# ylongqi/openrec

Measured on NVIDIA H100. Metric: bpr_triplets_per_sec, higher is better.
Workload: dtype f32

## Files before the change

### openrec_b200/csrc/orx_common.cuh

```cuda
#pragma once
#include <cuda_runtime.h>
#include <stdint.h>
#include <stdio.h>

#include <functional>
#include <initializer_list>
#include <type_traits>

#include "../../include/orx.h"

void orx_set_error(const char* fmt, ...);

#define ORX_CUDA(call)                                                                         \
  do {                                                                                         \
    cudaError_t e__ = (call);                                                                  \
    if (e__ != cudaSuccess) {                                                                  \
      orx_set_error("%s:%d %s -> %s", __FILE__, __LINE__, #call, cudaGetErrorString(e__));     \
      return ORX_ERR_CUDA;                                                                     \
    }                                                                                          \
  } while (0)

#define ORX_REQUIRE(cond, msg)                                  \
  do {                                                          \
    if (!(cond)) {                                              \
// ... 237 lines not shown
  return r;
}
__device__ __forceinline__ float orx_rcp_fast(float x) {
  float r;
  asm("rcp.approx.f32 %0, %1;" : "=f"(r) : "f"(x));
  return r;
}

template <int OPT>
struct OrxOptSlots {
  static constexpr bool S0 = (OPT == ORX_OPT_ADAGRAD || OPT == ORX_OPT_ADAM_LAZY);
  static constexpr bool S1 = (OPT == ORX_OPT_ADAM_LAZY);
  static constexpr bool STAGE_ONLY = (OPT == ORX_OPT_ADAM_DENSE);
};

template <int OPT>
__device__ __forceinline__ float orx_apply(float w, float g, float& s0, float& s1, const OrxOptDev& o) {
  if (OPT == ORX_OPT_SGD) {
    return w - o.lr * g;
  } else if (OPT == ORX_OPT_ADAGRAD) {
    s0 = s0 + g * g;
    return w - o.lr * g * orx_rcp_fast(orx_sqrt_fast(s0) + o.eps);
  } else {
    s0 = o.beta1 * s0 + (1.f - o.beta1) * g;
    s1 = o.beta2 * s1 + (1.f - o.beta2) * g * g;
    return w - o.lr * s0 * orx_rcp_fast(orx_sqrt_fast(s1) + o.eps);
  }
}

template <int OPT>
__device__ __forceinline__ float4 orx_apply4(float4 w, float4 g, float4& s0, float4& s1, const OrxOptDev& o) {
  float4 r;
  r.x = orx_apply<OPT>(w.x, g.x, s0.x, s1.x, o);
  r.y = orx_apply<OPT>(w.y, g.y, s0.y, s1.y, o);
  r.z = orx_apply<OPT>(w.z, g.z, s0.z, s1.z, o);
  r.w = orx_apply<OPT>(w.w, g.w, s0.w, s1.w, o);
  return r;
}

template <int OPT, bool STREAM>
__device__ __forceinline__ void orx_own_or_stage4(bool own, float* W, float* P0, float* P1, int id, float* G, int d,
                                                  int D, int off, float4 w, float4 g, float4& s0, float4& s1,
                                                  const OrxOptDev& o) {
  typedef OrxOptSlots<OPT> SL;
  auto st = [](float* p, float4 v) {
    if (STREAM) orx_st4_stream(p, v);
    else __stcg(reinterpret_cast<float4*>(p), v);
  };
  if (!SL::STAGE_ONLY && own) {
    const int64_t i = (int64_t)id * D + off;
    st(W + i, orx_apply4<OPT>(w, g, s0, s1, o));
    if (SL::S0) st(P0 + i, s0);
    if (SL::S1) st(P1 + i, s1);
  } else {
    orx_red4(G + (int64_t)d * D + off, g);
  }
}

template <int OPT>
__device__ __forceinline__ void orx_update1(float* W, float* P0, float* P1, float w, float g, const OrxOptDev& o) {
  typedef OrxOptSlots<OPT> SL;
  float s0 = SL::S0 ? *P0 : 0.f, s1 = SL::S1 ? *P1 : 0.f;
  *W = orx_apply<OPT>(w, g, s0, s1, o);
  if (SL::S0) *P0 = s0;
  if (SL::S1) *P1 = s1;
}

__device__ __forceinline__ void orx_adam_dense1(float* W, float* M, float* V, int64_t i, float g, const OrxOptDev& o) {
  const float mm = o.beta1 * M[i] + (1.f - o.beta1) * g;
  const float vv = o.beta2 * V[i] + (1.f - o.beta2) * g * g;
  M[i] = mm;
  V[i] = vv;
  W[i] = W[i] - o.lr * mm / (sqrtf(vv) + o.eps);
}

__device__ __forceinline__ void orx_block_partial(float loss, float l2, float* partials) {
  __shared__ float sred[8][2];
  loss = orx_group_sum<32>(loss);
  l2 = orx_group_sum<32>(l2);
  if ((threadIdx.x & 31) == 0) {
    sred[threadIdx.x >> 5][0] = loss;
    sred[threadIdx.x >> 5][1] = l2;
  }
  __syncthreads();
  if (threadIdx.x == 0) {
    float l = 0.f, q = 0.f;
#pragma unroll
    for (int w = 0; w < 8; ++w) {
      l += sred[w][0];
      q += sred[w][1];
    }
    partials[2 * blockIdx.x] = l;
    partials[2 * blockIdx.x + 1] = q;
  }
}

__device__ __forceinline__ void orx_warp_partial(float loss, float l2, float* partials) {
  const int warp = (blockIdx.x * blockDim.x + threadIdx.x) >> 5;
  loss = orx_group_sum<32>(loss);
  l2 = orx_group_sum<32>(l2);
  if ((threadIdx.x & 31) == 0) {
    partials[2 * warp] = loss;
    partials[2 * warp + 1] = l2;
  }
}

__device__ __forceinline__ void orx_block_sum_partials(const float* partials, int n, const float* sq, int nsq,
                                                       double* l, double* q) {
  __shared__ double sh[2][256];
  double sl = 0.0, sq2 = 0.0;
  for (int i = threadIdx.x; i < n; i += blockDim.x) {
    sl += (double)__ldcg(partials + 2 * i);
    sq2 += (double)__ldcg(partials + 2 * i + 1);
  }
  if (sq)
    for (int e = threadIdx.x; e < nsq; e += blockDim.x) sq2 += (double)sq[e] * (double)sq[e];
  sh[0][threadIdx.x] = sl;
  sh[1][threadIdx.x] = sq2;
  __syncthreads();
  for (int s = 128; s > 0; s >>= 1) {
    if ((int)threadIdx.x < s) {
      sh[0][threadIdx.x] += sh[0][threadIdx.x + s];
      sh[1][threadIdx.x] += sh[1][threadIdx.x + s];
    }
    __syncthreads();
  }
  *l = sh[0][0];
  *q = sh[1][0];
}

#endif

struct SparseArgs {
  float *U, *Us0, *Us1;
  float *I, *Is0, *Is1;
  float *Bv, *Bs0, *Bs1;
  float *gu, *gi, *gb;
  OrxHash hu, hi;
  OrxOptDev opt;
  int D;
};

struct TailArgs : SparseArgs {
  const float* partials;
  int n_partials;
  float loss_scale;
  int32_t* counters;
  float* out4;
  float *W, *Ws0, *Ws1, *gw;
  float c_l2;
};

#ifdef __CUDACC__
template <int OPT>
__device__ __forceinline__ void orx_tail_rows(const TailArgs& a, int nu, int ni) {
  typedef OrxOptSlots<OPT> SL;
  constexpr bool ZERO_ONLY = SL::STAGE_ONLY;
  const int lane = threadIdx.x & 31;
  const int gwarp = (blockIdx.x * blockDim.x + threadIdx.x) >> 5;
  const int nwarps = (gridDim.x * blockDim.x) >> 5;
  const int D = a.D;
  const float4 z4 = make_float4(0.f, 0.f, 0.f, 0.f);
  const int sub = lane >> 3, sl = lane & 7;
  for (int r0 = gwarp * 4; r0 < nu + ni; r0 += nwarps * 4) {
    const int r = r0 + sub;
    const bool on = r < nu + ni;
    const bool is_u = on && r < nu;
    const int d = on ? (is_u ? r : r - nu) : 0;
    const int id = on ? (is_u ? a.hu.did[d] : a.hi.did[d]) : 0;
    float* G = (is_u ? a.gu : a.gi) + (int64_t)d * D;
    float* W = (is_u ? a.U : a.I) + (int64_t)id * D;
    float* P0 = (is_u ? a.Us0 : a.Is0) + (int64_t)id * D;
    float* P1 = (is_u ? a.Us1 : a.Is1) + (int64_t)id * D;
    if ((D & 3) == 0) {
      const int nq = D >> 2;
      for (int e0 = 0; e0 < nq; e0 += 32) {
        float4 g[4], w[4], s0v[4], s1v[4];
#pragma unroll
        for (int k = 0; k < 4; ++k) {
          const int e = e0 + sl + 8 * k;
          const bool ld = on && e < nq;
          g[k] = ld ? __ldcg(reinterpret_cast<const float4*>(G) + e) : z4;
          w[k] = (ld && !ZERO_ONLY) ? orx_ld4_stream(W + 4 * e) : z4;
          s0v[k] = (ld && SL::S0) ? orx_ld4_stream(P0 + 4 * e) : z4;
          s1v[k] = (ld && SL::S1) ? orx_ld4_stream(P1 + 4 * e) : z4;
        }
#pragma unroll
        for (int k = 0; k < 4; ++k) {
          const int e = e0 + sl + 8 * k;
          if (!on || e >= nq) continue;
          if (!ZERO_ONLY) {
            orx_st4_stream(W + 4 * e, orx_apply4<OPT>(w[k], g[k], s0v[k], s1v[k], a.opt));
            if (SL::S0) orx_st4_stream(P0 + 4 * e, s0v[k]);
            if (SL::S1) orx_st4_stream(P1 + 4 * e, s1v[k]);
          }
          __stcg(reinterpret_cast<float4*>(G) + e, z4);
        }
      }
    } else if (on) {
      for (int e = sl; e < D; e += 8) {
        if (!ZERO_ONLY) orx_update1<OPT>(W + e, P0 + e, P1 + e, W[e], G[e], a.opt);
        G[e] = 0.f;
      }
    }
    if (on && !is_u && sl == 0) {
      if (!ZERO_ONLY) orx_update1<OPT>(a.Bv + id, a.Bs0 + id, a.Bs1 + id, a.Bv[id], a.gb[d], a.opt);
      a.gb[d] = 0.f;
    }
  }
}
#endif

OrxOptDev orx_opt_to_dev(const orx_opt_t* o);
int orx_launch_index_build_strided(orx_ctx* c, const int32_t* a, int64_t stride, int64_t rows, int32_t n,
                                   bool stage_all, cudaStream_t st);
SparseArgs orx_sparse_args(const orx_ctx* c, const orx_table_t* user, const orx_table_t* item, const orx_table_t* bias,
                           const OrxHash& hu, const OrxHash& hi, const OrxOptDev& o);
int orx_check_step_tables(const orx_table_t* user, const orx_table_t* item, const orx_table_t* bias,
                          const orx_table_t* w, int opt_kind);
static inline int orx_step_blocks(int B) { return ((B + 7) / 8 + 7) / 8; }
struct OrxStepLaunch {
  int n_partials, variant, minb;
};
typedef std::function<int(const SparseArgs& s, float* partials, OrxStepLaunch* out)> OrxStepKernel;
int orx_sparse_step(orx_ctx* c, int op, int kind, const orx_table_t* user, const orx_table_t* item,
                    const orx_table_t* bias, const orx_table_t* w, const int32_t* uid, const int32_t* iid,
                    const int32_t* nid, int B, const orx_opt_t* opt, float loss_scale, float c_l2, float* out4,
                    const OrxStepKernel& kernel, cudaStream_t st);
int orx_sparse_unfused(orx_ctx* c, int B, float loss_scale, float* out4,
                       const std::function<void(float* partials, int blocks)>& launch, cudaStream_t st);
int orx_launch_adam_sweeps(orx_ctx* c, const orx_table_t* user, const orx_table_t* item, const orx_table_t* bias,
                           const OrxHash& hu, const OrxHash& hi, const OrxOptDev& o, cudaStream_t st);
int orx_launch_tail(orx_ctx* c, const TailArgs& ta, int opt_kind, cudaStream_t st);
int orx_launch_reduce_partials(const float* partials, int n, float loss_scale, float* out4, cudaStream_t st);
int orx_launch_index_build(orx_ctx* c, const int32_t* a, int64_t rows_a, const int32_t* b0, const int32_t* b1,
                           int64_t rows_b, int32_t n, int mode , cudaStream_t st);
```

### openrec_b200/csrc/orx_pairwise.cu

```cuda
#include "orx_common.cuh"
#include "orx_pair.cuh"

__global__ void k_index_build(OrxHash hu, OrxHash hi, const int32_t* __restrict__ a, int64_t rows_a,
                              const int32_t* __restrict__ b0, const int32_t* __restrict__ b1, int64_t rows_b, int n,
                              int stage_all, int32_t* bad) {
  const int i = blockIdx.x * blockDim.x + threadIdx.x;
  if (i >= (b1 ? 3 : 2) * n) return;
  const int t = i < n ? i : (i < 2 * n ? i - n : i - 2 * n);
  const int32_t ia = a[t], ib0 = b0[t], ib1 = b1 ? b1[t] : 0;
  const bool ga = ia >= 0 && (int64_t)ia < rows_a, gb0 = ib0 >= 0 && (int64_t)ib0 < rows_b,
             gb1 = ib1 >= 0 && (int64_t)ib1 < rows_b;
  const bool all = ga && gb0 && gb1;
  if (i < n) {
    if (!ga) atomicAdd(bad, 1);
    else if (all) orx_hash_insert(hu, ia, stage_all);
  } else {
    const bool g = i < 2 * n ? gb0 : gb1;
    if (!g) atomicAdd(bad, 1);
    else if (all) orx_hash_insert(hi, i < 2 * n ? ib0 : ib1, stage_all);
  }
}

__global__ void k_index_build_strided(OrxHash hu, const int32_t* __restrict__ a, int64_t stride, int64_t rows, int n,
                                       int stage_all, int32_t* bad) {
// ... 186 lines not shown
  } else {
#pragma unroll 1
    for (int j = 0; j < CH; j += TPW) {
      if (j > 0) {
        load_var(j, ra);
        load_slots(j, ra);
      }
      process(j, ra);
    }
  }

  orx_pdl_trigger();
  if (flags & 1) {
    if (flags & 4) {
      __stcg(a.Bv + p_id, orx_apply<OPT>(bp, g_own, bps0, bps1, a.opt));
      if (SL::S0) __stcg(a.Bs0 + p_id, bps0);
      if (SL::S1) __stcg(a.Bs1 + p_id, bps1);
    } else {
      atomicAdd(a.gb + dp, g_own);
    }
    if (flags & 8) {
      __stcg(a.Bv + n_id, orx_apply<OPT>(bn, -g_own, bns0, bns1, a.opt));
      if (SL::S0) __stcg(a.Bs0 + n_id, bns0);
      if (SL::S1) __stcg(a.Bs1 + n_id, bns1);
    } else {
      atomicAdd(a.gb + dn, -g_own);
    }
  }

  orx_block_partial(loss_acc, l2_acc, a.partials);
}

template <int KIND, int OPT, int MODE>
__global__ void __launch_bounds__(256) k_pair_generic(const PairArgs a) {
  constexpr bool STAGE_ONLY = OrxOptSlots<OPT>::STAGE_ONLY;
  const int lane = threadIdx.x & 31;
  const int warp = (blockIdx.x * blockDim.x + threadIdx.x) >> 5;
  const int D = a.D;
  const bool row_form = MODE == 1 && a.ld != 0;
  const int64_t ld = row_form ? a.ld : D;
  float loss_acc = 0.f, l2_acc = 0.f;
  orx_pdl_wait();
  for (int j = 0; j < 8; ++j) {
    const int t = warp * 8 + j;
    if (t >= a.B) break;
    const int uu = a.uid[t], pp = a.pid[t], nn = a.nid[t];
    const bool ok = uu >= 0 && uu < a.rowsU && pp >= 0 && pp < a.rowsI && nn >= 0 && nn < a.rowsI;
    float* ur = a.U + (int64_t)uu * ld;
    float* pr = a.I + (int64_t)pp * ld;
    float* nr = a.I + (int64_t)nn * ld;
    float s1 = 0.f, s2 = 0.f, sq = 0.f, bp = 0.f, bn = 0.f, lt = 0.f, g = 0.f;
    if (ok) {
      for (int d = lane; d < D; d += 32) {
        const float u = ur[d], p = pr[d], n = nr[d];
        if (KIND == ORX_PAIR_BPR) {
          s1 += u * p;
          s2 += u * n;
        } else {
          s1 += (u - p) * (u - p);
          s2 += (u - n) * (u - n);
        }
        sq += u * u + p * p + n * n;
      }
      bp = row_form ? pr[D] : a.Bv[pp];
      bn = row_form ? nr[D] : a.Bv[nn];
    }
    l2_acc += sq;
    s1 = orx_group_sum<32>(s1);
    s2 = orx_group_sum<32>(s2);
    if (ok) pair_score<KIND>(s1, s2, bp, bn, a.margin, a.c_loss, a.inv_B, &lt, &g);
    if (lane == 0) loss_acc += lt;
    const float gbias = (KIND == ORX_PAIR_BPR) ? g : -g;
    if (MODE == 0) {
      if (!ok) continue;
      int du, dp, dn;
      const uint32_t cu = orx_hash_find<!STAGE_ONLY>(a.hu, uu, &du);
      const uint32_t cp = orx_hash_find<!STAGE_ONLY>(a.hi, pp, &dp);
      const uint32_t cn = orx_hash_find<!STAGE_ONLY>(a.hi, nn, &dn);
      const bool fu = !STAGE_ONLY && cu == 1u, fp = !STAGE_ONLY && cp == 1u, fn = !STAGE_ONLY && cn == 1u;
      for (int d = lane; d < D; d += 32) {
        const float u = ur[d], p = pr[d], n = nr[d];
        float gu, gp, gn;
        pair_grads1<KIND>(g, a.c_l2, u, p, n, &gu, &gp, &gn);
        const int64_t ou = (int64_t)uu * D + d, op = (int64_t)pp * D + d, on = (int64_t)nn * D + d;
        if (fu) orx_update1<OPT>(ur + d, a.Us0 + ou, a.Us1 + ou, u, gu, a.opt);
        else atomicAdd(a.gu + (int64_t)du * D + d, gu);
        if (fp) orx_update1<OPT>(pr + d, a.Is0 + op, a.Is1 + op, p, gp, a.opt);
        else atomicAdd(a.gi + (int64_t)dp * D + d, gp);
        if (fn) orx_update1<OPT>(nr + d, a.Is0 + on, a.Is1 + on, n, gn, a.opt);
        else atomicAdd(a.gi + (int64_t)dn * D + d, gn);
      }
      if (lane == 0) {
        if (fp) orx_update1<OPT>(a.Bv + pp, a.Bs0 + pp, a.Bs1 + pp, bp, gbias, a.opt);
        else atomicAdd(a.gb + dp, gbias);
        if (fn) orx_update1<OPT>(a.Bv + nn, a.Bs0 + nn, a.Bs1 + nn, bn, -gbias, a.opt);
        else atomicAdd(a.gb + dn, -gbias);
      }
      continue;
    }
    if (a.d_user || a.d_pos || a.d_neg) {
      for (int d = lane; d < D; d += 32) {
        float gu = 0.f, gp = 0.f, gn = 0.f;
        if (ok) pair_grads1<KIND>(g, a.c_l2, ur[d], pr[d], nr[d], &gu, &gp, &gn);
        if (row_form) {
          if (ok) {
            a.d_user[(int64_t)uu * ld + d] = gu;
            a.d_pos[(int64_t)pp * ld + d] = gp;
            a.d_neg[(int64_t)nn * ld + d] = gn;
          }
        } else {
          const int64_t o = (int64_t)t * D + d;
          if (a.d_user) a.d_user[o] = gu;
          if (a.d_pos) a.d_pos[o] = gp;
          if (a.d_neg) a.d_neg[o] = gn;
        }
      }
    }
    if (lane == 0) {
      if (row_form) {
        if (ok) {
          for (int64_t c = D; c < ld; ++c) {
            a.d_user[(int64_t)uu * ld + c] = 0.f;
            a.d_pos[(int64_t)pp * ld + c] = c == D ? gbias : 0.f;
            a.d_neg[(int64_t)nn * ld + c] = c == D ? -gbias : 0.f;
          }
        }
      } else {
        if (a.d_bp) a.d_bp[t] = gbias;
        if (a.d_bn) a.d_bn[t] = -gbias;
      }
      if (a.g_out) a.g_out[t] = g;
    }
  }
  orx_warp_partial(loss_acc, l2_acc, a.partials);
}

__global__ void __launch_bounds__(256) k_adam_sweep(float* var, float* m, float* v, int64_t rows, int D, OrxHash h,
                                                    const float* gstage, OrxOptDev o) {
  const int lane = threadIdx.x & 31;
  const int64_t nw = ((int64_t)gridDim.x * blockDim.x) >> 5;
  for (int64_t r = ((int64_t)blockIdx.x * blockDim.x + threadIdx.x) >> 5; r < rows; r += nw) {
    int d = -1;
    uint32_t c = 0;
    if (lane == 0) c = orx_hash_find(h, (int32_t)r, &d);
    c = __shfl_sync(ORX_FULL, c, 0);
    d = __shfl_sync(ORX_FULL, d, 0);
    for (int e = lane; e < D; e += 32)
      orx_adam_dense1(var, m, v, r * D + e, c ? gstage[(int64_t)d * D + e] : 0.f, o);
  }
}


template <int OPT>
__global__ void __launch_bounds__(256) k_sparse_tail(const TailArgs a) {
  __shared__ bool last;
  orx_pdl_wait();
  const int nu = *a.hu.counter, ni = a.I ? *a.hi.counter : 0;
  orx_tail_rows<OPT>(a, nu, ni);

  if (blockIdx.x == 0 && a.out4) {
    double l, q;
    orx_block_sum_partials(a.partials, a.n_partials, a.W, a.W ? a.D : 0, &l, &q);
    if (threadIdx.x == 0) {
      a.out4[0] = (float)(l * (double)a.loss_scale);
      a.out4[1] = (float)(0.5 * q);
      a.out4[2] = (float)a.counters[3];
      a.out4[3] = (float)(nu + ni);
    }
    if (a.W) {
      for (int e = threadIdx.x; e < a.D; e += blockDim.x) {
        const float g = a.gw[e] + a.c_l2 * a.W[e];
        if (OrxOptSlots<OPT>::STAGE_ONLY) orx_adam_dense1(a.W, a.Ws0, a.Ws1, e, g, a.opt);
        else orx_update1<OPT>(a.W + e, a.Ws0 + e, a.Ws1 + e, a.W[e], g, a.opt);
        a.gw[e] = 0.f;
      }
    }
  }
  __syncthreads();
  if (threadIdx.x == 0) {
    __threadfence();
    const int tk = atomicAdd(a.counters + 2, 1);
    last = (tk == (int)gridDim.x - 1);
  }
  __syncthreads();
  if (last && threadIdx.x < 4) a.counters[threadIdx.x] = 0;
}

int orx_launch_tail(orx_ctx* c, const TailArgs& ta, int opt_kind, cudaStream_t st) {
  const int grid = c->num_sms * 4;
  orx_dispatch_opt(opt_kind, [&](auto O) {
    orx_launch_pdl(k_sparse_tail<decltype(O)::value>, dim3(grid), dim3(256), 0, st, ta);
  });
  ORX_LAUNCH_CHECK();
  return ORX_OK;
}

int orx_launch_adam_sweeps(orx_ctx* c, const orx_table_t* user, const orx_table_t* item, const orx_table_t* bias,
                           const OrxHash& hu, const OrxHash& hi, const OrxOptDev& o, cudaStream_t st) {
  struct { const orx_table_t* t; int D; const OrxHash* h; const float* g; } sw[3] = {
      {user, user->dim, &hu, c->gu}, {item, user->dim, &hi, c->gi}, {bias, 1, &hi, c->gb}};
  for (const auto& s : sw) {
    if (!s.t) continue;
    int64_t blocks = (s.t->rows + 7) / 8;
    const int64_t cap = (int64_t)c->num_sms * 16;
    if (blocks > cap) blocks = cap;
    if (blocks < 1) blocks = 1;
    k_adam_sweep<<<(int)blocks, 256, 0, st>>>(s.t->var, s.t->s0, s.t->s1, s.t->rows, s.D, *s.h, s.g, o);
    ORX_LAUNCH_CHECK();
  }
  return ORX_OK;
}

SparseArgs orx_sparse_args(const orx_ctx* c, const orx_table_t* user, const orx_table_t* item, const orx_table_t* bias,
                           const OrxHash& hu, const OrxHash& hi, const OrxOptDev& o) {
  SparseArgs s = {};
  s.U = user->var; s.Us0 = user->s0; s.Us1 = user->s1;
  if (item) { s.I = item->var; s.Is0 = item->s0; s.Is1 = item->s1; }
  if (bias) { s.Bv = bias->var; s.Bs0 = bias->s0; s.Bs1 = bias->s1; }
  s.D = user->dim; s.opt = o; s.hu = hu; s.hi = hi;
  s.gu = c->gu; s.gi = c->gi; s.gb = c->gb;
  return s;
}

int orx_check_step_tables(const orx_table_t* user, const orx_table_t* item, const orx_table_t* bias,
                          const orx_table_t* w, int opt_kind) {
  ORX_REQUIRE(user && item && bias, "null table");
  ORX_REQUIRE(user->var && item->var && bias->var, "null table storage");
  ORX_REQUIRE(user->dim == item->dim && user->dim > 0, "user/item dims must match and be positive");
  ORX_REQUIRE(bias->dim == 1 && bias->rows == item->rows, "item_bias must be [item.rows, 1]");
  ORX_REQUIRE(user->rows > 0 && item->rows > 0 && user->rows <= 0x7fffffffLL && item->rows <= 0x7fffffffLL,
              "row counts must fit int32 ids");
  ORX_REQUIRE(!w || (w->var && w->dim == user->dim), "GMF needs w with dim == D");
  ORX_REQUIRE(orx_opt_slots_ok(opt_kind, {user, item, bias, w}), "optimizer slot rows missing");
  return ORX_OK;
}

template <int KIND, int OPT>
static int launch_pair_step_kind_opt(const PairArgs& pa, cudaStream_t st, OrxStepLaunch* out) {
  constexpr bool LAZY = (OPT == ORX_OPT_ADAM_LAZY);
  const int blocks = orx_step_blocks(pa.B);
  auto go = [&](auto kern, int variant, int minb, int n_partials) {
    *out = {n_partials, variant, minb};
    orx_launch_pdl(kern, dim3(blocks), dim3(256), 0, st, pa);
  };
  constexpr int PV = LAZY ? ORX_VARIANT_STEP : ORX_VARIANT_STEP_PIPE;
  switch (pa.D) {
    case 32: go(k_pair_step<KIND, OPT, 32, 8, 2, !LAZY>, PV, 2, blocks); break;
    case 64: go(k_pair_step<KIND, OPT, 64, 8, 2, !LAZY>, PV, 2, blocks); break;
    case 128:
      if constexpr (LAZY) go(k_pair_step<KIND, OPT, 128, 8, 3, false>, ORX_VARIANT_STEP, 3, blocks);
      else go(k_pair_step<KIND, OPT, 128, 8, 4, false>, ORX_VARIANT_STEP, 4, blocks);
      break;
    case 256: go(k_pair_step<KIND, OPT, 256, 8, 2, !LAZY>, PV, 2, blocks); break;
    default: go(k_pair_generic<KIND, OPT, 0>, ORX_VARIANT_STEP_GENERIC, 0, 8 * blocks); break;
  }
  ORX_LAUNCH_CHECK();
  return ORX_OK;
}

static int side_stream_ensure(orx_ctx* c) {
  if (c->side_stream) return ORX_OK;
  ORX_CUDA(cudaStreamCreateWithFlags(&c->side_stream, cudaStreamNonBlocking));
  ORX_CUDA(cudaEventCreateWithFlags(&c->side_ev, cudaEventDisableTiming));
  for (int i = 0; i < 2; ++i) {
    ORX_CUDA(cudaEventCreateWithFlags(&c->pf_done[i], cudaEventDisableTiming));
    ORX_CUDA(cudaEventCreateWithFlags(&c->pf_free[i], cudaEventDisableTiming));
    ORX_CUDA(cudaEventCreateWithFlags(&c->stage_free[i], cudaEventDisableTiming));
    c->pf_free_valid[i] = c->stage_free_valid[i] = 0;
  }
  return ORX_OK;
}

static int prefetch_drop(orx_ctx* c, cudaStream_t st) {
  if (!c->pf_valid) return ORX_OK;
  const int k = c->pf_set;
  ORX_CUDA(cudaStreamWaitEvent(st, c->pf_done[k], 0));
  ORX_CUDA(cudaMemsetAsync(c->counters + 4 * (1 + k), 0, sizeof(int32_t) * 4, st));
  ORX_CUDA(cudaEventRecord(c->pf_free[k], st));
  c->pf_free_valid[k] = 1;
  c->pf_valid = 0;
  return ORX_OK;
}

static int prefetch_issue(orx_ctx* c, const int32_t* uid, const int32_t* pid, const int32_t* nid, int B, int64_t rows_u,
                          int64_t rows_i, int mode) {
  const int k = c->pf_next;
  c->pf_next ^= 1;
  cudaStream_t ss = c->side_stream;
  if (c->pf_free_valid[k]) ORX_CUDA(cudaStreamWaitEvent(ss, c->pf_free[k], 0));
  int rc = orx_next_epoch(c, ss);
  if (rc) return rc;
  c->pf_u[k].epoch = c->pf_i[k].epoch = c->epoch;
  k_index_build<<<(3 * B + 255) / 256, 256, 0, ss>>>(c->pf_u[k], c->pf_i[k], uid, rows_u, pid, nid, rows_i, B, mode,
                                                     c->counters + 4 * (1 + k) + 3);
  ORX_LAUNCH_CHECK();
  ORX_CUDA(cudaEventRecord(c->pf_done[k], ss));
  c->pf_valid = 1; c->pf_set = k; c->pf_uid = uid; c->pf_pid = pid; c->pf_nid = nid; c->pf_B = B;
  c->pf_rows_u = rows_u; c->pf_rows_i = rows_i; c->pf_mode = mode;
  return ORX_OK;
}

extern "C" int orx_pairwise_prefetch(orx_handle_t h, const orx_table_t* user, const orx_table_t* item, const int32_t* uid,
                                     const int32_t* pid, const int32_t* nid, int32_t B, int32_t opt_kind, int32_t ids_ready,
                                     orx_stream_t ids_stream) {
  ORX_REQUIRE(h != nullptr && user && item && uid && pid && nid && B > 0, "bad arguments");
  ORX_REQUIRE(orx_opt_kind_ok(opt_kind), "unknown optimizer kind");
  ORX_REQUIRE(!orx_shard_holds_index(h), "a sharded step's announced batch holds this handle's index sets (a prefetch "
                                         "would overwrite one) until its orx_shard_step call");
  ORX_CUDA(cudaSetDevice(h->device));
  cudaStream_t is = (cudaStream_t)ids_stream;
  int rc = orx_ensure_workspace(h, B, user->dim);
  if (rc) return rc;
  if ((rc = side_stream_ensure(h))) return rc;
  if ((rc = prefetch_drop(h, is))) return rc;
  if (!ids_ready) {
    ORX_CUDA(cudaEventRecord(h->side_ev, is));
    ORX_CUDA(cudaStreamWaitEvent(h->side_stream, h->side_ev, 0));
  }
  return prefetch_issue(h, uid, pid, nid, B, user->rows, item->rows, opt_kind == ORX_OPT_ADAM_DENSE ? 1 : 0);
}

int orx_sparse_step(orx_ctx* c, int op, int kind, const orx_table_t* user, const orx_table_t* item,
                    const orx_table_t* bias, const orx_table_t* w, const int32_t* uid, const int32_t* iid,
                    const int32_t* nid, int B, const orx_opt_t* opt, float loss_scale, float c_l2, float* out4,
                    const OrxStepKernel& kernel, cudaStream_t st) {
  ORX_REQUIRE(opt != nullptr && out4 != nullptr, "null opt/out");
  ORX_REQUIRE(orx_opt_kind_ok(opt->kind), "unknown optimizer kind");
  ORX_REQUIRE(B > 0 && uid && iid, "empty batch or null ids");
  int rc = orx_check_step_tables(user, item, bias, w, opt->kind);
  if (rc) return rc;
  const int D = user->dim;
  if ((rc = orx_ensure_workspace(c, B, D))) return rc;
  const bool dense = opt->kind == ORX_OPT_ADAM_DENSE;
  if ((rc = orx_grow((void**)&c->partials, &c->partials_cap, sizeof(float) * 2 * 8 * (size_t)orx_step_blocks(B))))
    return rc;
  orx_prof_mark(c, 0, st);
  int set = 0;
  if (nid && c->pf_valid && c->pf_uid == uid && c->pf_pid == iid && c->pf_nid == nid && c->pf_B == B &&
      c->pf_rows_u == user->rows && c->pf_rows_i == item->rows && c->pf_mode == (dense ? 1 : 0)) {
    set = 1 + c->pf_set;
    ORX_CUDA(cudaStreamWaitEvent(st, c->pf_done[c->pf_set], 0));
    c->pf_valid = 0;
  } else {
    if (nid && (rc = prefetch_drop(c, st))) return rc;
// ... 189 lines not shown
```

### openrec_b200/csrc/orx_shard.cu

```cuda
#include <stdlib.h>
#include <string.h>

#include "orx_common.cuh"
#include "orx_pair.cuh"

#define SH_MAX_R 64
#define SH_META 16
#define SH_NPH 4
#define SH_ERR_WORD (SH_NPH * SH_MAX_R)
#define SH_IDX_BITS 24

enum { SH_M_TRIPS = 0,
       SH_M_REQS = 1,
       SH_M_GOTOFF = 2,
       SH_M_GINBASE = 3,
       SH_M_LOSS = 4, SH_M_L2 = 5 };

enum { SH_C_CURH = 0, SH_C_CURO = SH_MAX_R, SH_C_GOFF = 2 * SH_MAX_R, SH_C_RCO = 3 * SH_MAX_R + 1,
       SH_C_DONE = 4 * SH_MAX_R + 1, SH_C_T = SH_C_DONE + 8, SH_C_NREQ = SH_C_T + 1, SH_C_ACUR = SH_C_T + 2,
       SH_C_BAD = SH_C_T + 4 , SH_C_WORDS = SH_C_T + 8 };

struct ShardHost {
  int32_t world, rank, dim, batch_cap, home_cap, req_cap, gin_cap, timeout_ms;
  void *tripbox, *idbox, *got, *gotb, *gin, *ginb, *meta, *flags;
// ... 424 lines not shown
        }
        sq += dot4(u[k][q], u[k][q]) + dot4(p[k][q], p[k][q]) + dot4(n[k][q], n[k][q]);
      }
      l2_acc += sq;
      s1 = orx_group_sum<32>(s1);
      s2 = orx_group_sum<32>(s2);
      const float bp = __shfl_sync(ORX_FULL, my_bp, k), bn = __shfl_sync(ORX_FULL, my_bn, k);
      float lt, g;
      pair_score<KIND>(s1, s2, bp, bn, a.margin, a.c_loss, a.inv_B, &lt, &g);
      if (lane == 0) loss_acc += lt;
      const int own = __shfl_sync(ORX_FULL, my_own, k);
      const int du = __shfl_sync(ORX_FULL, my_du, k);
      float* dp = reinterpret_cast<float*>(__shfl_sync(ORX_FULL, (unsigned long long)my_dp, k));
      float* dn = reinterpret_cast<float*>(__shfl_sync(ORX_FULL, (unsigned long long)my_dn, k));
      const int pp = __shfl_sync(ORX_FULL, my_pp, k), pn = __shfl_sync(ORX_FULL, my_pn, k);
#pragma unroll
      for (int q = 0; q < NQ; ++q) {
        const int e = q * 32 + lane;
        if (e >= nq) continue;
        float4 gu, gp, gn;
        pair_row_grads<KIND>(g, a.c_l2, u[k][q], p[k][q], n[k][q], &gu, &gp, &gn);
        if (dp) reinterpret_cast<float4*>(dp)[e] = gp;
        if (dn) reinterpret_cast<float4*>(dn)[e] = gn;
        orx_own_or_stage4<OPT, false>(own, a.U, a.Us0, a.Us1, uu[k], a.gu, du, D, 4 * e, u[k][q], gu, us0[k][q],
                                      us1[k][q], a.opt);
      }
      {
        float* bdp = reinterpret_cast<float*>(__shfl_sync(ORX_FULL, (unsigned long long)my_bdp, k));
        float* bdn = reinterpret_cast<float*>(__shfl_sync(ORX_FULL, (unsigned long long)my_bdn, k));
        const float gb = (KIND == ORX_PAIR_BPR) ? g : -g;
        if (lane == 0) {
          if (bdp) *bdp = gb;
          if (bdn) *bdn = -gb;
        }
      }
    }
  }
  orx_pdl_trigger();
  orx_warp_partial(loss_acc, l2_acc, a.partials);
  sh_arrive(x, w.ctl + SH_C_DONE + 3, gridDim.x, 3, epoch, [&]() {
    double l, q;
    orx_block_sum_partials(a.partials, (int)((gridDim.x * blockDim.x) >> 5), nullptr, 0, &l, &q);
    if ((int)threadIdx.x < R) {
      int32_t* m = x.meta[threadIdx.x] + SH_META * me;
      m[SH_M_LOSS] = __float_as_int((float)(l * (double)a.loss_scale));
      m[SH_M_L2] = __float_as_int((float)(0.5 * q));
    }
  });
}

struct ShApplyArgs {
  float *I, *Is0, *Is1;
  float *Bv, *Bs0, *Bs1;
  OrxHash hi;
  float *gi, *gb;
  OrxOptDev opt;
};

struct ShProArgs {
  int n_route, n_request;
  int epoch;
  ShRouteArgs r;
  OrxHash hu;
};

template <int OPT, int NQ>
__global__ void __launch_bounds__(256) k_sh_apply(ShardDev x, ShardWs w, ShApplyArgs a, ShProArgs pro, int epoch) {
  typedef OrxOptSlots<OPT> SL;
  constexpr int GRP = NQ == 1 ? 4 : (NQ == 2 ? 2 : 1);
  const int me = x.rank, D = x.D, nq = D >> 2;
  orx_pdl_wait();
  if ((int)blockIdx.x < pro.n_route) {
    sh_route_role(x, w, pro.r, pro.epoch, blockIdx.x, pro.n_route);
    orx_pdl_trigger();
    return;
  }
  if ((int)blockIdx.x < pro.n_route + pro.n_request) {
    sh_request_role(x, w, pro.hu, pro.epoch, blockIdx.x - pro.n_route, pro.n_request);
    orx_pdl_trigger();
    return;
  }
  sh_wait(x, 3, epoch);
  const int n = w.ctl[SH_C_NREQ];
  const int lane = threadIdx.x & 31, wid = threadIdx.x >> 5;
  const float* gin = x.gin[me];
  const float* ginb = x.ginb[me];
  const float4 z4 = make_float4(0.f, 0.f, 0.f, 0.f);
  __shared__ int chunk_sh;
  while (true) {
    __syncthreads();
    if (threadIdx.x == 0) chunk_sh = atomicAdd(w.ctl + SH_C_ACUR, 1);
    __syncthreads();
    const int j0 = chunk_sh * 64 + wid * 8;
    if (chunk_sh * 64 >= n) break;
    if (j0 >= n) continue;
    int32_t my_id = -1;
    int my_d = -1, my_own = 0;
    if (lane < 8) {
      my_id = w.req[j0 + lane];
      if (my_id >= 0) {
        my_own = orx_hash_find(a.hi, my_id, &my_d) == 1u;
        const float gbv = __ldcg(ginb + j0 + lane);
        if (my_own) {
          float s0v = SL::S0 ? __ldcg(a.Bs0 + my_id) : 0.f, s1v = SL::S1 ? __ldcg(a.Bs1 + my_id) : 0.f;
          __stcg(a.Bv + my_id, orx_apply<OPT>(__ldcg(a.Bv + my_id), gbv, s0v, s1v, a.opt));
          if (SL::S0) __stcg(a.Bs0 + my_id, s0v);
          if (SL::S1) __stcg(a.Bs1 + my_id, s1v);
        } else {
          atomicAdd(a.gb + my_d, gbv);
        }
      }
    }
    if (__ballot_sync(ORX_FULL, my_id >= 0) == 0u) continue;
#pragma unroll
    for (int k0 = 0; k0 < 8; k0 += GRP) {
      float4 g[GRP][NQ], wv[GRP][NQ], s0v[GRP][NQ], s1v[GRP][NQ];
      int id[GRP], own[GRP], d[GRP];
#pragma unroll
      for (int k = 0; k < GRP; ++k) {
        id[k] = __shfl_sync(ORX_FULL, my_id, k0 + k);
        own[k] = __shfl_sync(ORX_FULL, my_own, k0 + k);
        d[k] = __shfl_sync(ORX_FULL, my_d, k0 + k);
#pragma unroll
        for (int q = 0; q < NQ; ++q) {
          const int e = q * 32 + lane;
          const bool on = id[k] >= 0 && e < nq;
          g[k][q] = on ? __ldcg(reinterpret_cast<const float4*>(gin + (int64_t)(j0 + k0 + k) * D) + e) : z4;
          const bool ld = on && own[k];
          wv[k][q] = ld ? __ldcg(reinterpret_cast<const float4*>(a.I + (int64_t)id[k] * D) + e) : z4;
          s0v[k][q] = (SL::S0 && ld) ? __ldcg(reinterpret_cast<const float4*>(a.Is0 + (int64_t)id[k] * D) + e) : z4;
          s1v[k][q] = (SL::S1 && ld) ? __ldcg(reinterpret_cast<const float4*>(a.Is1 + (int64_t)id[k] * D) + e) : z4;
        }
      }
#pragma unroll
      for (int k = 0; k < GRP; ++k) {
        if (id[k] < 0) continue;
#pragma unroll
        for (int q = 0; q < NQ; ++q) {
          const int e = q * 32 + lane;
          if (e >= nq) continue;
          orx_own_or_stage4<OPT, false>(own[k], a.I, a.Is0, a.Is1, id[k], a.gi, d[k], D, 4 * e, wv[k][q], g[k][q],
                                        s0v[k][q], s1v[k][q], a.opt);
        }
      }
    }
  }
  orx_pdl_trigger();
}

template <int OPT>
__global__ void __launch_bounds__(256) k_sh_tail(ShardDev x, ShardWs w, TailArgs a, int par) {
  orx_pdl_wait();
  const int nu = *a.hu.counter, ni = *a.hi.counter;
  orx_tail_rows<OPT>(a, nu, ni);
  if (blockIdx.x == 0 && threadIdx.x == 0) {
    const int32_t* m = x.meta[x.rank];
    float l = 0.f, q = 0.f;
    for (int r = 0; r < x.world; ++r) {
      l += __int_as_float(__ldcg(m + SH_META * r + SH_M_LOSS));
      q += __int_as_float(__ldcg(m + SH_META * r + SH_M_L2));
    }
    a.out4[0] = l;
    a.out4[1] = q;
    a.out4[2] = (float)w.ctl[SH_C_BAD + par];
    a.out4[3] = (float)(nu + ni);
    w.ctl[SH_C_BAD + par] = 0;
    w.ctl[SH_C_ACUR] = 0;
  }
  __shared__ bool last;
  __syncthreads();
  if (threadIdx.x == 0) {
    __threadfence();
    last = (atomicAdd(a.counters + 2, 1) == (int)gridDim.x - 1);
  }
  __syncthreads();
  if (last && threadIdx.x == 0) {
    *a.hu.counter = 0;
    *a.hi.counter = 0;
    a.counters[2] = 0;
  }
}

struct orx_shard_ws {
  ShardWs w;
  int home_cap, gin_cap, got_rows;
  const void* occ_fn[32];
  int occ[32], n_occ;
  int32_t pro_route[2], pro_request[2];
  uint32_t ep_u[2], ep_i[2];
  const int32_t *ids_u[2], *ids_p[2], *ids_n[2];
  int32_t ids_B[2];
  int32_t serve_epoch, tail_epoch;
  const void* owner;
};

extern "C" int orx_peer_alloc(orx_handle_t h, int64_t bytes, void** dev_ptr_out, uint8_t* handle_out64) {
  ORX_REQUIRE(h != nullptr && dev_ptr_out && handle_out64 && bytes > 0, "bad arguments");
  ORX_CUDA(cudaSetDevice(h->device));
  void* p = nullptr;
  ORX_CUDA(cudaMalloc(&p, (size_t)bytes));
  ORX_CUDA(cudaMemset(p, 0, (size_t)bytes));
  ORX_CUDA(cudaDeviceSynchronize());
  cudaIpcMemHandle_t hd;
  static_assert(sizeof(cudaIpcMemHandle_t) == 64, "IPC handle size");
  ORX_CUDA(cudaIpcGetMemHandle(&hd, p));
  memcpy(handle_out64, &hd, 64);
  *dev_ptr_out = p;
  return ORX_OK;
}

extern "C" int orx_peer_open(orx_handle_t h, const uint8_t* handle64, void** dev_ptr_out) {
  ORX_REQUIRE(h != nullptr && dev_ptr_out && handle64, "bad arguments");
  ORX_CUDA(cudaSetDevice(h->device));
  cudaIpcMemHandle_t hd;
  memcpy(&hd, handle64, 64);
  void* p = nullptr;
  ORX_CUDA(cudaIpcOpenMemHandle(&p, hd, cudaIpcMemLazyEnablePeerAccess));
  *dev_ptr_out = p;
  return ORX_OK;
}

extern "C" int orx_peer_close(orx_handle_t h, void* dev_ptr) {
  ORX_REQUIRE(h != nullptr, "null handle");
  if (dev_ptr) ORX_CUDA(cudaIpcCloseMemHandle(dev_ptr));
  return ORX_OK;
}

extern "C" int orx_peer_free(orx_handle_t h, void* dev_ptr) {
  ORX_REQUIRE(h != nullptr, "null handle");
  if (dev_ptr) ORX_CUDA(cudaFree(dev_ptr));
  return ORX_OK;
}

static int sh_ctas_per_sm(orx_shard_ws* s, const void* fn, int cap) {
  for (int i = 0; i < s->n_occ; ++i)
    if (s->occ_fn[i] == fn) return s->occ[i] < cap ? s->occ[i] : cap;
  int nb = 0;
  if (cudaOccupancyMaxActiveBlocksPerMultiprocessor(&nb, fn, 256, 0) != cudaSuccess || nb < 1) nb = 1;
  if (s->n_occ < 32) { s->occ_fn[s->n_occ] = fn; s->occ[s->n_occ++] = nb; }
  return nb < cap ? nb : cap;
}

static size_t sh_layout(char* base, int home_cap, int gin_cap, ShardWs* w) {
  size_t off = 0;
  auto take = [&](size_t words) {
    int32_t* p = base ? reinterpret_cast<int32_t*>(base + off) : nullptr;
    off += (sizeof(int32_t) * words + 255) & ~(size_t)255;
    return p;
  };
  w->trip_u = take((size_t)home_cap);
  w->slot = take(2 * (size_t)home_cap);
  w->req = take((size_t)gin_cap);
  w->ctl = take(SH_C_WORDS);
  return off;
}

void orx_shard_ws_release(orx_ctx* c) {
  delete (orx_shard_ws*)c->shard_ws;
  c->shard_ws = nullptr;
}

bool orx_shard_holds_index(const orx_ctx* c) {
  const orx_shard_ws* s = (const orx_shard_ws*)c->shard_ws;
  return s && (s->pro_route[0] > s->tail_epoch || s->pro_route[1] > s->tail_epoch);
}

static int shard_ws_ensure(orx_ctx* c, const ShardHost* x, cudaStream_t st) {
  orx_shard_ws* s = (orx_shard_ws*)c->shard_ws;
  const int got_rows = sh_got_rows(x->home_cap, x->world);
  if (s && s->home_cap >= x->home_cap && s->gin_cap >= x->gin_cap && s->got_rows >= got_rows) return ORX_OK;
  orx_shard_ws_release(c);
  c->shard_ws = s = new orx_shard_ws();
  int rc = orx_grow(&c->shard_scratch, &c->shard_cap, sh_layout(nullptr, x->home_cap, x->gin_cap, &s->w));
  if (rc) return rc;
  sh_layout(static_cast<char*>(c->shard_scratch), x->home_cap, x->gin_cap, &s->w);
  ORX_CUDA(cudaMemsetAsync(s->w.ctl, 0, sizeof(int32_t) * SH_C_WORDS, st));
  s->home_cap = x->home_cap;
  s->gin_cap = x->gin_cap;
  s->got_rows = got_rows;
  return ORX_OK;
}

static int shard_check(orx_handle_t h, const ShardHost* x) {
  ORX_REQUIRE(h != nullptr && x != nullptr, "null handle / descriptor");
  ORX_REQUIRE(x->world >= 1 && x->world <= SH_MAX_R && x->rank >= 0 && x->rank < x->world, "bad world / rank");
  ORX_REQUIRE(x->dim >= 4 && (x->dim & 3) == 0 && x->dim <= 512, "dim must be a multiple of 4 in [4, 512]");
  ORX_REQUIRE(x->batch_cap > 0 && x->home_cap > 0 && x->req_cap > 0 && x->gin_cap >= 32 && x->timeout_ms > 0, "bad capacities");
  ORX_REQUIRE(x->req_cap < (1 << SH_IDX_BITS), "req_cap must stay below 2^24");
  ORX_REQUIRE(x->tripbox && x->idbox && x->got && x->gotb && x->gin && x->ginb && x->meta && x->flags, "null mailbox pointer table");
  return ORX_OK;
}

static ShardDev shard_to_dev(const ShardHost* x) {
  ShardDev d;
  d.world = x->world; d.rank = x->rank; d.D = x->dim; d.batch_cap = x->batch_cap; d.home_cap = x->home_cap;
  d.req_cap = x->req_cap; d.gin_cap = x->gin_cap; d.got_rows = sh_got_rows(x->home_cap, x->world);
  d.timeout_ns = (unsigned long long)x->timeout_ms * 1000000ull;
  d.tripbox = (int32_t* const*)x->tripbox; d.idbox = (int32_t* const*)x->idbox;
  d.got = (float* const*)x->got; d.gotb = (float* const*)x->gotb;
  d.gin = (float* const*)x->gin; d.ginb = (float* const*)x->ginb;
  d.meta = (int32_t* const*)x->meta; d.flags = (int32_t* const*)x->flags;
  return d;
}

extern "C" int orx_shard_sizes(const orx_shard_t* xs, int64_t* n8_host) {
  const ShardHost* x = (const ShardHost*)xs;
  ORX_REQUIRE(x != nullptr && n8_host != nullptr, "null pointer");
// ... 189 lines not shown
```

Baseline: 358.6 million.

## Prefetch first tail rows before PDL wait and resize tail grid per optimizer

The sparse tail kernel now reads the hash counters and row ids, and prefetches the first batch of weight, optimizer-slot and bias values, before calling the PDL wait. This overlaps those loads with the end of the preceding step kernel instead of stalling on them afterward. The grid drops from 4 CTAs per SM to 2 or 3 depending on optimizer slot count, with matching launch bounds, and the loss reduction moves to the last block. The risk is that early reads before the dependency wait could see stale data if the previous kernel writes those rows or counters.

```diff
diff --git a/openrec_b200/csrc/orx_common.cuh b/openrec_b200/csrc/orx_common.cuh
--- a/openrec_b200/csrc/orx_common.cuh
+++ b/openrec_b200/csrc/orx_common.cuh
@@ -413,7 +413,7 @@
 };
 
 #ifdef __CUDACC__
-template <int OPT>
+template <int OPT, bool EARLY>
 __device__ __forceinline__ void orx_tail_rows(const TailArgs& a, int nu, int ni) {
   typedef OrxOptSlots<OPT> SL;
   constexpr bool ZERO_ONLY = SL::STAGE_ONLY;
@@ -423,28 +423,41 @@
   const int D = a.D;
   const float4 z4 = make_float4(0.f, 0.f, 0.f, 0.f);
   const int sub = lane >> 3, sl = lane & 7;
-  for (int r0 = gwarp * 4; r0 < nu + ni; r0 += nwarps * 4) {
+  const int nq = D >> 2;
+  auto row_of = [&](int r0, bool& on, bool& is_u, int& d, int& id) {
     const int r = r0 + sub;
-    const bool on = r < nu + ni;
-    const bool is_u = on && r < nu;
-    const int d = on ? (is_u ? r : r - nu) : 0;
-    const int id = on ? (is_u ? a.hu.did[d] : a.hi.did[d]) : 0;
+    on = r < nu + ni;
+    is_u = on && r < nu;
+    d = on ? (is_u ? r : r - nu) : 0;
+    id = on ? __ldcg(is_u ? a.hu.did + d : a.hi.did + d) : 0;
+  };
+  auto load_rows = [&](bool on, bool is_u, int id, int e0, float4* w, float4* s0v, float4* s1v) {
+    const float* W = (is_u ? a.U : a.I) + (int64_t)id * D;
+    const float* P0 = (is_u ? a.Us0 : a.Is0) + (int64_t)id * D;
+    const float* P1 = (is_u ? a.Us1 : a.Is1) + (int64_t)id * D;
+#pragma unroll
+    for (int k = 0; k < 4; ++k) {
+      const int e = e0 + sl + 8 * k;
+      const bool ld = on && e < nq;
+      w[k] = (ld && !ZERO_ONLY) ? orx_ld4_stream(W + 4 * e) : z4;
+      s0v[k] = (ld && SL::S0) ? orx_ld4_stream(P0 + 4 * e) : z4;
+      s1v[k] = (ld && SL::S1) ? orx_ld4_stream(P1 + 4 * e) : z4;
+    }
+  };
+  auto apply_row = [&](bool PRE, bool on, bool is_u, int d, int id, float4* w, float4* s0v, float4* s1v, float bw,
+                       float bs0, float bs1) {
     float* G = (is_u ? a.gu : a.gi) + (int64_t)d * D;
     float* W = (is_u ? a.U : a.I) + (int64_t)id * D;
     float* P0 = (is_u ? a.Us0 : a.Is0) + (int64_t)id * D;
     float* P1 = (is_u ? a.Us1 : a.Is1) + (int64_t)id * D;
     if ((D & 3) == 0) {
-      const int nq = D >> 2;
       for (int e0 = 0; e0 < nq; e0 += 32) {
-        float4 g[4], w[4], s0v[4], s1v[4];
+        float4 g[4];
+        if (!PRE || e0 > 0) load_rows(on, is_u, id, e0, w, s0v, s1v);
 #pragma unroll
         for (int k = 0; k < 4; ++k) {
           const int e = e0 + sl + 8 * k;
-          const bool ld = on && e < nq;
-          g[k] = ld ? __ldcg(reinterpret_cast<const float4*>(G) + e) : z4;
-          w[k] = (ld && !ZERO_ONLY) ? orx_ld4_stream(W + 4 * e) : z4;
-          s0v[k] = (ld && SL::S0) ? orx_ld4_stream(P0 + 4 * e) : z4;
-          s1v[k] = (ld && SL::S1) ? orx_ld4_stream(P1 + 4 * e) : z4;
+          g[k] = (on && e < nq) ? __ldcg(reinterpret_cast<const float4*>(G) + e) : z4;
         }
 #pragma unroll
         for (int k = 0; k < 4; ++k) {
@@ -465,9 +478,49 @@
       }
     }
     if (on && !is_u && sl == 0) {
-      if (!ZERO_ONLY) orx_update1<OPT>(a.Bv + id, a.Bs0 + id, a.Bs1 + id, a.Bv[id], a.gb[d], a.opt);
+      if (!ZERO_ONLY) {
+        if (!PRE) {
+          bw = a.Bv[id];
+          if (SL::S0) bs0 = a.Bs0[id];
+          if (SL::S1) bs1 = a.Bs1[id];
+        }
+        a.Bv[id] = orx_apply<OPT>(bw, a.gb[d], bs0, bs1, a.opt);
+        if (SL::S0) a.Bs0[id] = bs0;
+        if (SL::S1) a.Bs1[id] = bs1;
+      }
       a.gb[d] = 0.f;
     }
+  };
+
+  int r0 = gwarp * 4;
+  if (EARLY) {
+    bool on, is_u;
+    int d, id;
+    row_of(r0, on, is_u, d, id);
+    float4 w[4], s0v[4], s1v[4];
+    float bw = 0.f, bs0 = 0.f, bs1 = 0.f;
+    const bool pre = (D & 3) == 0;
+    if (pre) {
+      load_rows(on, is_u, id, 0, w, s0v, s1v);
+      if (on && !is_u && sl == 0 && !ZERO_ONLY) {
+        bw = __ldcg(a.Bv + id);
+        if (SL::S0) bs0 = __ldcg(a.Bs0 + id);
+        if (SL::S1) bs1 = __ldcg(a.Bs1 + id);
+      }
+    }
+    orx_pdl_wait();
+    if (r0 < nu + ni) {
+      if (pre) apply_row(true, on, is_u, d, id, w, s0v, s1v, bw, bs0, bs1);
+      else apply_row(false, on, is_u, d, id, w, s0v, s1v, 0.f, 0.f, 0.f);
+    }
+    r0 += nwarps * 4;
+  }
+  for (; r0 < nu + ni; r0 += nwarps * 4) {
+    bool on, is_u;
+    int d, id;
+    row_of(r0, on, is_u, d, id);
+    float4 w[4], s0v[4], s1v[4];
+    apply_row(false, on, is_u, d, id, w, s0v, s1v, 0.f, 0.f, 0.f);
   }
 }
 #endif
diff --git a/openrec_b200/csrc/orx_pairwise.cu b/openrec_b200/csrc/orx_pairwise.cu
--- a/openrec_b200/csrc/orx_pairwise.cu
+++ b/openrec_b200/csrc/orx_pairwise.cu
@@ -362,13 +362,16 @@
 
 
 template <int OPT>
-__global__ void __launch_bounds__(256) k_sparse_tail(const TailArgs a) {
+struct TailShape {
+  static constexpr int CTAS_PER_SM = OrxOptSlots<OPT>::S1 ? 2 : 3;
+};
+template <int OPT>
+__global__ void __launch_bounds__(256, TailShape<OPT>::CTAS_PER_SM) k_sparse_tail(const TailArgs a) {
   __shared__ bool last;
-  orx_pdl_wait();
-  const int nu = *a.hu.counter, ni = a.I ? *a.hi.counter : 0;
-  orx_tail_rows<OPT>(a, nu, ni);
-
-  if (blockIdx.x == 0 && a.out4) {
+  const int nu = __ldcg(a.hu.counter), ni = a.I ? __ldcg(a.hi.counter) : 0;
+  orx_tail_rows<OPT, true>(a, nu, ni);
+
+  if (blockIdx.x == gridDim.x - 1 && a.out4) {
     double l, q;
     orx_block_sum_partials(a.partials, a.n_partials, a.W, a.W ? a.D : 0, &l, &q);
     if (threadIdx.x == 0) {
@@ -397,9 +400,9 @@
 }
 
 int orx_launch_tail(orx_ctx* c, const TailArgs& ta, int opt_kind, cudaStream_t st) {
-  const int grid = c->num_sms * 4;
   orx_dispatch_opt(opt_kind, [&](auto O) {
-    orx_launch_pdl(k_sparse_tail<decltype(O)::value>, dim3(grid), dim3(256), 0, st, ta);
+    constexpr int OPT = decltype(O)::value;
+    orx_launch_pdl(k_sparse_tail<OPT>, dim3(c->num_sms * TailShape<OPT>::CTAS_PER_SM), dim3(256), 0, st, ta);
   });
   ORX_LAUNCH_CHECK();
   return ORX_OK;
diff --git a/openrec_b200/csrc/orx_shard.cu b/openrec_b200/csrc/orx_shard.cu
--- a/openrec_b200/csrc/orx_shard.cu
+++ b/openrec_b200/csrc/orx_shard.cu
@@ -600,7 +600,7 @@
 __global__ void __launch_bounds__(256) k_sh_tail(ShardDev x, ShardWs w, TailArgs a, int par) {
   orx_pdl_wait();
   const int nu = *a.hu.counter, ni = *a.hi.counter;
-  orx_tail_rows<OPT>(a, nu, ni);
+  orx_tail_rows<OPT, false>(a, nu, ni);
   if (blockIdx.x == 0 && threadIdx.x == 0) {
     const int32_t* m = x.meta[x.rank];
     float l = 0.f, q = 0.f;
```

New measurement: 365.5 million (median of 6 runs). 1.9% higher.
